# AaltoML/free-hunch

Measured on AMD Instinct MI355X. Metric: images/sec (256x256, num_steps=30, FH-Heun), higher is better.
Workload: dtype f32 UNet (convolutions: exact 3-way bf16 split on the bf16 MFMA, fp32 accuracy) + f64 covariance/CG; 1 GPU; FFHQ-256 arch, gaussian_blur, FH low-rank covariance (dct_diagonal), num_steps=30 heun, batch=8 per GPU; lockstep_groups_per_gpu=2, unet_backend=hip, net_calls_per_image=59

## Files before the change

free-hunch_amd/_lib.py:

```python
from __future__ import annotations

import ctypes as C
import os

import torch

_HERE = os.path.dirname(os.path.abspath(__file__))
LIB_PATH = os.path.join(_HERE, "libfh_hip.so")

c_dp = C.c_void_p


class FhProblem(C.Structure):
    _fields_ = [("op", C.c_int32), ("use_dct", C.c_int32), ("planes", C.c_int32), ("stride", C.c_int32),
                ("ntaps", C.c_int32), ("m", C.c_int32), ("ldm", C.c_int32), ("halo", C.c_int32),
                ("d", C.c_int64), ("sigma_y2", C.c_double),
                ("tap_dy", c_dp), ("tap_dx", c_dp), ("tap_w", c_dp), ("mask", c_dp),
                ("D", c_dp), ("r", c_dp), ("B", c_dp), ("M", c_dp),
                ("ntaps2", C.c_int32), ("halo2", C.c_int32), ("cg_scipy", C.c_int32), ("fold_sym", C.c_int32),
                ("tap2_dy", c_dp), ("tap2_dx", c_dp), ("tap2_w", c_dp),
                ("fold_fwd_w", c_dp), ("fold_fwd_h", c_dp), ("fold_inv_w", c_dp), ("fold_inv_h", c_dp)]


FH_MAX_BATCH = 16
# ... 56 lines not shown
    "fh_amm": ([C.c_void_p, C.POINTER(FhProblem), c_dp, c_dp, C.c_void_p], C.c_int),
    "fh_dense_matvec_scratch_doubles": ([C.c_int, C.c_int64], C.c_int64),
    "fh_dense_matvec": ([c_dp, c_dp, c_dp, c_dp, C.c_int, C.c_int64, C.c_int, C.c_double, C.c_double, C.c_void_p], C.c_int),
    "fh_dense_rank2": ([c_dp, c_dp, C.c_int, C.c_int64, c_dp, c_dp, c_dp, c_dp, c_dp, c_dp, C.c_double, C.c_double,
                        C.c_void_p], C.c_int),
    "fh_conv2d_nhwc": ([c_dp, c_dp, c_dp, c_dp, c_dp, c_dp] + [C.c_int] * 10 + [C.c_void_p], C.c_int),
    "fh_conv2d_x6_nhwc": ([c_dp, c_dp, c_dp, c_dp, c_dp, c_dp] + [C.c_int] * 10 + [C.c_void_p], C.c_int),
    "fh_conv2d_x6_nhwc_gn": ([c_dp, c_dp, c_dp, c_dp, c_dp, c_dp] + [C.c_int] * 10 + [C.POINTER(FhGnEpilogue), C.c_void_p],
                             C.c_int),
    "fh_conv2d_x6_gn_chunks": ([C.c_int] * 10, C.c_int),
    "fh_groupnorm_finalize": ([c_dp, c_dp, C.c_int, C.c_int, C.c_double, C.c_int, C.c_void_p], C.c_int),
    "fh_groupnorm_bwd_table": ([c_dp, c_dp, c_dp, c_dp, c_dp, C.c_int, c_dp, C.c_int, C.c_int, C.c_void_p], C.c_int),
    "fh_groupnorm_bwd_apply": ([c_dp] * 8 + [C.c_int, c_dp] + [C.c_int] * 5 + [C.c_void_p], C.c_int),
    "fh_groupnorm_bwd_sums": ([c_dp] * 7 + [C.c_int, c_dp, c_dp] + [C.c_int] * 4 + [C.c_void_p], C.c_int),
    "fh_groupnorm_bwd_apply_ex": ([c_dp] * 8 + [C.c_int, c_dp, c_dp, c_dp, c_dp] + [C.c_int] * 5 + [c_dp, C.c_void_p], C.c_int),
    "fh_conv2d_splitk": ([C.c_int] * 7, C.c_int),
    "fh_unet_set_precision": ([C.c_int], C.c_int),
    "fh_unet_get_precision": ([], C.c_int),
    "fh_absmax_f32": ([c_dp, C.c_int64, c_dp, C.c_void_p], C.c_int),
    "fh_groupnorm_table": ([c_dp, c_dp, c_dp, c_dp, c_dp, C.c_int, c_dp, C.c_int, C.c_int, C.c_void_p], C.c_int),
    "fh_conv2d_x6_norm_supported": ([C.c_int] * 5, C.c_int),
    "fh_conv2d_x6_norm_nhwc": ([c_dp, c_dp, C.c_int, c_dp, c_dp, c_dp, c_dp] + [C.c_int] * 5 + [C.c_void_p], C.c_int),
    "fh_conv2d_x6_norm_nhwc_gn": ([c_dp, c_dp, C.c_int, c_dp, c_dp, c_dp, c_dp] + [C.c_int] * 5
                                  + [C.POINTER(FhGnEpilogue), C.c_void_p], C.c_int),
    "fh_conv3x3_thin_nhwc": ([c_dp, c_dp, c_dp, c_dp] + [C.c_int] * 5 + [C.c_void_p], C.c_int),
    "fh_conv3x3_wino_nhwc": ([c_dp, c_dp, c_dp, c_dp, c_dp] + [C.c_int] * 5 + [C.c_void_p], C.c_int),
    "fh_bgemm_f32": ([c_dp, c_dp, c_dp] + [C.c_int] * 10 + [C.c_int64] * 6 + [C.c_float, C.c_void_p], C.c_int),
    "fh_groupnorm_scratch_doubles": ([C.c_int, C.c_int], C.c_int64),
    "fh_groupnorm_stats": ([c_dp, c_dp, c_dp, C.c_int, C.c_int, C.c_int, C.c_void_p], C.c_int),
    "fh_groupnorm_apply": ([c_dp] * 6 + [C.c_int, c_dp, C.c_int, C.c_int, C.c_int, C.c_int, C.c_void_p], C.c_int),
# ... 138 lines not shown
```

free-hunch_amd/csrc/fh_unet.hip:

```cpp
#include "fh_common.h"
#include <stdlib.h>

typedef float float16_t __attribute__((ext_vector_type(16)));

namespace {

constexpr int kBK = 32;
constexpr int kLd = kBK + 4;

struct ConvArgs {
  const float* in;
  const float* w;
  const float* bias;
  const float* res;
  float* out;
  int N, H, W, Cin, Cout, KH, KW, pad, stride, Ho, Wo;
  int ksplit;
  float* ws;
};

__device__ __forceinline__ void xcd_tile(int& tile_m, int& tile_n) {
  const unsigned gx = gridDim.x, gy = gridDim.y;
  const unsigned total = gx * gy;
  unsigned lin = blockIdx.y * gx + blockIdx.x;
// ... 1052 lines not shown
  if (col < g.N) {
#pragma unroll
    for (int r = 0; r < 16; ++r) {
      const int row = m0 + wm + (r & 3) + 8 * (r >> 2) + 4 * lh;
      if (row < g.M) C[(int64_t)row * g.ldc + col] = g.alpha * acc[r];
    }
  }
}

static inline int gn_chunk(int N, int P) {
  int c = 512;
  while (c > 32 && (int64_t)N * ((P + c - 1) / c) < 256) c >>= 1;
  return c;
}

template <int MODE>
__global__ __launch_bounds__(256) void k_gn_partial(const float* __restrict__ x, const float* __restrict__ dy,
                                                    const float* __restrict__ stats, const float* __restrict__ gamma,
                                                    const float* __restrict__ beta, const float* __restrict__ scale,
                                                    const float* __restrict__ shift, int ss_stride,
                                                    double* __restrict__ partial, int P, int C, int act, int nchunks,
                                                    int kGnChunk) {
  __shared__ double acc[64];
  const int n = blockIdx.x / nchunks, chunk = blockIdx.x % nchunks;
  const int cg = C / 32, c4n = C / 4;
  if (threadIdx.x < 64) acc[threadIdx.x] = 0.0;
  __syncthreads();
  const int p0 = chunk * kGnChunk;
  const int p1 = p0 + kGnChunk < P ? p0 + kGnChunk : P;
  const int lanes_p = c4n >= 256 ? 1 : 256 / c4n;
  const int active = c4n >= 256 ? 256 : lanes_p * c4n;
  if ((int)threadIdx.x < active) {
    for (int c4 = threadIdx.x % (c4n < 256 ? c4n : 256); c4 < c4n; c4 += 256) {
      const int psub = c4n >= 256 ? 0 : threadIdx.x / c4n;
      double s0[4] = {0, 0, 0, 0}, s1[4] = {0, 0, 0, 0};
      float ga[4], be[4], sc[4], sh[4], mean[4], rstd[4];
      if (MODE == 1) {
#pragma unroll
        for (int e = 0; e < 4; ++e) {
          const int c = 4 * c4 + e;
          ga[e] = gamma[c], be[e] = beta[c];
          sc[e] = scale != nullptr ? 1.f + scale[(int64_t)n * ss_stride + c] : 1.f;
          sh[e] = shift != nullptr ? shift[(int64_t)n * ss_stride + c] : 0.f;
          mean[e] = stats[((int64_t)n * 32 + c / cg) * 2], rstd[e] = stats[((int64_t)n * 32 + c / cg) * 2 + 1];
        }
      }
      for (int pb = p0 + psub; pb < p1; pb += 4 * lanes_p) {
        float4 xv[4], gv[4];
        bool ok[4];
#pragma unroll
        for (int u = 0; u < 4; ++u) {
          const int p = pb + u * lanes_p;
          ok[u] = p < p1;
          const int64_t idx = ((int64_t)n * P + (ok[u] ? p : p0)) * C + 4 * c4;
          xv[u] = *reinterpret_cast<const float4*>(x + idx);
          if (MODE == 1) gv[u] = *reinterpret_cast<const float4*>(dy + idx);
        }
#pragma unroll
        for (int u = 0; u < 4; ++u) {
          if (!ok[u]) continue;
          const float xs[4] = {xv[u].x, xv[u].y, xv[u].z, xv[u].w};
          if (MODE == 0) {
#pragma unroll
            for (int e = 0; e < 4; ++e) {
              s0[e] += xs[e];
              s1[e] += (double)xs[e] * xs[e];
            }
          } else {
            const float gs[4] = {gv[u].x, gv[u].y, gv[u].z, gv[u].w};
#pragma unroll
            for (int e = 0; e < 4; ++e) {
              const float xh = (xs[e] - mean[e]) * rstd[e];
              const float t = (xh * ga[e] + be[e]) * sc[e] + sh[e];
              float g = gs[e];
// ... 40 lines not shown
  for (int g = 0; g < 16; ++g) s += red[g][slot];
  const int grp = slot >> 1, which = slot & 1;
  const double other = __shfl_xor(s, 1, 64);
  if (MODE == 1) {
    out[((int64_t)n * 32 + grp) * 2 + which] = (float)(s / count);
  } else {
    const double sum = which ? other : s, sq = which ? s : other;
    const double mean = sum / count;
    double var = sq / count - mean * mean;
    var = var < 0 ? 0 : var;
    out[((int64_t)n * 32 + grp) * 2 + which] = which ? (float)(1.0 / sqrt(var + 1e-5)) : (float)mean;
  }
}


typedef float f4v_t __attribute__((ext_vector_type(4)));
__device__ __forceinline__ float4 ld_stream(const float* p, int nt) {
  if (nt) {
    const f4v_t v = __builtin_nontemporal_load(reinterpret_cast<const f4v_t*>(p));
    return make_float4(v.x, v.y, v.z, v.w);
  }
  return *reinterpret_cast<const float4*>(p);
}

template <int BWD, bool AMAX = false>
__global__ __launch_bounds__(256) void k_gn_stream(const float* __restrict__ x, const float* __restrict__ dy,
                                                   const float* __restrict__ stats, const float* __restrict__ sums,
                                                   const float* __restrict__ gamma, const float* __restrict__ beta,
                                                   const float* __restrict__ scale, const float* __restrict__ shift,
                                                   int ss_stride, float* __restrict__ out, int P, int C, int act,
                                                   int accumulate, int nchunks, int kGnChunk,
                                                   const float* __restrict__ acc_src = nullptr,
                                                   const float* __restrict__ add2 = nullptr, float* __restrict__ out2 = nullptr,
                                                   int csplit = 0, unsigned* __restrict__ amax = nullptr, int nt = 0) {
  unsigned mx0 = 0u, mx1 = 0u;
  const int n = blockIdx.x / nchunks, chunk = blockIdx.x % nchunks;
  const int cg = C / 32, c4n = C / 4;
  const int p0 = chunk * kGnChunk;
  const int p1 = p0 + kGnChunk < P ? p0 + kGnChunk : P;
  const int lanes_p = c4n >= 256 ? 1 : 256 / c4n;
  const int active = c4n >= 256 ? 256 : lanes_p * c4n;
  const bool live = (int)threadIdx.x < active;
  if (!live && !(BWD && AMAX)) return;
  for (int c4 = threadIdx.x % (c4n < 256 ? c4n : 256); live && c4 < c4n; c4 += 256) {
    const int psub = c4n >= 256 ? 0 : threadIdx.x / c4n;
    float A[4], Bc[4], mean[4], rstd[4], gsc[4], sa[4], sb[4];
#pragma unroll
    for (int e = 0; e < 4; ++e) {
      const int c = 4 * c4 + e;
      const int64_t si = ((int64_t)n * 32 + c / cg) * 2;
      mean[e] = stats[si], rstd[e] = stats[si + 1];
      const float sc = scale != nullptr ? 1.f + scale[(int64_t)n * ss_stride + c] : 1.f;
      const float sh = shift != nullptr ? shift[(int64_t)n * ss_stride + c] : 0.f;
      const float rg = rstd[e] * gamma[c];
      A[e] = rg * sc;
      Bc[e] = (beta[c] - mean[e] * rg) * sc + sh;
      gsc[e] = sc * gamma[c];
      if (BWD) sa[e] = sums[si], sb[e] = sums[si + 1];
    }
    for (int pb = p0 + psub; pb < p1; pb += 4 * lanes_p) {
      float4 xv[4], gv[4], ov[4];
      bool ok[4];
#pragma unroll
      for (int u = 0; u < 4; ++u) {
        const int p = pb + u * lanes_p;
        ok[u] = p < p1;
        const int64_t idx = ((int64_t)n * P + (ok[u] ? p : p0)) * C + 4 * c4;
        xv[u] = *reinterpret_cast<const float4*>(x + idx);
        if (BWD) {
          gv[u] = ld_stream(dy + idx, nt);
          if (accumulate) ov[u] = ld_stream((acc_src != nullptr ? acc_src : out) + idx, nt);
          if (add2 != nullptr) {
            const float4 t2 = ld_stream(add2 + idx, nt);
            if (accumulate)
              ov[u].x += t2.x, ov[u].y += t2.y, ov[u].z += t2.z, ov[u].w += t2.w;
            else
              ov[u] = t2;
          }
        }
      }
#pragma unroll
      for (int u = 0; u < 4; ++u) {
        if (!ok[u]) continue;
        const int64_t idx = ((int64_t)n * P + pb + u * lanes_p) * C + 4 * c4;
        const float xs[4] = {xv[u].x, xv[u].y, xv[u].z, xv[u].w};
        float o[4];
        if (!BWD) {
#pragma unroll
          for (int e = 0; e < 4; ++e) {
            const float t = fmaf(xs[e], A[e], Bc[e]);
            o[e] = act ? silu_f(t) : t;
          }
        } else {
          const float gs[4] = {gv[u].x, gv[u].y, gv[u].z, gv[u].w};
          const float os[4] = {ov[u].x, ov[u].y, ov[u].z, ov[u].w};
#pragma unroll
          for (int e = 0; e < 4; ++e) {
// ... 99 lines not shown
      reinterpret_cast<float4*>(out)[i] = v;
    }
  }
}

__global__ __launch_bounds__(256) void k_concat(float* __restrict__ a, float* __restrict__ b, float* __restrict__ out,
                                                int64_t P, int Ca, int Cb, int split) {
  const int C4 = (Ca + Cb) / 4, Ca4 = Ca / 4, Cb4 = Cb / 4;
  for (int64_t i = (int64_t)blockIdx.x * 256 + threadIdx.x; i < P * C4; i += (int64_t)gridDim.x * 256) {
    const int c4 = (int)(i % C4);
    const int64_t p = i / C4;
    float4* o = reinterpret_cast<float4*>(out) + i;
    float4* s = c4 < Ca4 ? reinterpret_cast<float4*>(a) + p * Ca4 + c4 : reinterpret_cast<float4*>(b) + p * Cb4 + (c4 - Ca4);
    if (split) *s = *o; else *o = *s;
  }
}

__global__ __launch_bounds__(256) void k_nchw_to_nhwc(const float* __restrict__ in, float* __restrict__ out, int N,
                                                      int C, int64_t P, int Cp) {
  for (int64_t i = (int64_t)blockIdx.x * 256 + threadIdx.x; i < (int64_t)N * P * Cp; i += (int64_t)gridDim.x * 256) {
    const int c = (int)(i % Cp);
    const int64_t p = (i / Cp) % P, n = i / (Cp * P);
    out[i] = c < C ? in[((int64_t)n * C + c) * P + p] : 0.f;
  }
}
__global__ __launch_bounds__(256) void k_nhwc_to_nchw(const float* __restrict__ in, float* __restrict__ out, int N,
                                                      int C, int64_t P, int Cp) {
  for (int64_t i = (int64_t)blockIdx.x * 256 + threadIdx.x; i < (int64_t)N * C * P; i += (int64_t)gridDim.x * 256) {
    const int64_t p = i % P;
    const int c = (int)((i / P) % C);
// ... 103 lines not shown
  }
  return false;
}

bool launch_x6_tile(const X6Plan& p, hipStream_t st, const ConvArgsX& a) {
  switch (tile_key(p.bm, p.bn)) {
    case tile_key(128, 128): launch_x6<2, 1, 2, 4, 4>(p, st, a); return true;
    case tile_key(64, 128): launch_x6<1, 2, 2, 2, 2>(p, st, a); return true;
    case tile_key(64, 64): launch_x6<1, 1, 2, 2, 2>(p, st, a); return true;
  }
  return false;
}

}

extern "C" {

int fh_unet_set_precision(int mode) {
  if (mode < 0 || mode > 4) return FH_EINVAL;
  g_conv_np = mode == 0 ? 3 : (mode == 1 ? 1 : (mode == 2 ? 2 : (mode == 3 ? 16 : 32)));
  return 0;
}

int fh_unet_get_precision(void) {
  return g_conv_np == 3 ? 0 : (g_conv_np == 1 ? 1 : (g_conv_np == 2 ? 2 : (g_conv_np == 16 ? 3 : 4)));
}

int fh_absmax_f32(const float* x, int64_t n, float* out, void* stream) {
  if (!out || n < 0 || (n > 0 && !x) || ((uintptr_t)x & 15)) return FH_EINVAL;
  hipStream_t st = (hipStream_t)stream;
// ... 335 lines not shown
  const int nchunks = (P + kGnChunk - 1) / kGnChunk;
  static const int nt_env = getenv("FH_GN_NT") ? atoi(getenv("FH_GN_NT")) : 1;
  const int nt = nt_env && (int64_t)N * P * C * 4 > ((int64_t)200 << 20);
  if (amax2 != nullptr)
    hipLaunchKernelGGL((k_gn_stream<1, true>), dim3(N * nchunks), dim3(256), 0, (hipStream_t)stream, x, dy, stats, sums, gamma,
                       beta, scale, shift, ss_stride, dx, P, C, act, acc_src != nullptr ? 1 : 0, nchunks, kGnChunk, acc_src, add2,
                       dx2, csplit, reinterpret_cast<unsigned*>(amax2), nt);
  else
    hipLaunchKernelGGL((k_gn_stream<1, false>), dim3(N * nchunks), dim3(256), 0, (hipStream_t)stream, x, dy, stats, sums, gamma,
                       beta, scale, shift, ss_stride, dx, P, C, act, acc_src != nullptr ? 1 : 0, nchunks, kGnChunk, acc_src, add2,
                       dx2, csplit, (unsigned*)nullptr, nt);
  FH_LAUNCH_CHECK();
  return 0;
}

int fh_softmax_rows(float* s, int64_t rows, int T, void* stream) {
  if (!s || rows < 1 || T < 1) return FH_EINVAL;
  hipLaunchKernelGGL(k_softmax_rows, dim3((unsigned)rows), dim3(256), 0, (hipStream_t)stream, s, T);
  FH_LAUNCH_CHECK();
  return 0;
}

int fh_softmax_bwd_rows(const float* p, float* dp, int64_t rows, int T, void* stream) {
  if (!p || !dp || rows < 1 || T < 1) return FH_EINVAL;
  hipLaunchKernelGGL(k_softmax_bwd_rows, dim3((unsigned)rows), dim3(256), 0, (hipStream_t)stream, p, dp, T);
  FH_LAUNCH_CHECK();
  return 0;
}

int fh_resample2x(const float* in, float* out, int N, int Hs, int Ws, int C, int mode, void* stream) {
// ... 36 lines not shown
```

free-hunch_amd/unet_hip.py:

```python
from __future__ import annotations

import math
import os
import threading

import torch
import torch.nn.functional as F

import ctypes as C

from . import _lib

_K = 32


def _pad_to(n, m):
    return (n + m - 1) // m * m


def _wino(w):
    w0, w1, w2 = w[:, :, 0], w[:, :, 1], w[:, :, 2]
    return torch.stack([w0, (w0 + w1 + w2) / 2, (w0 - w1 + w2) / 2, w2], 0).contiguous()


# ... 209 lines not shown
        e.partial, e.mode, e.act = partial.data_ptr(), mode, 0
        e.in_amax = None if amax is None else amax.data_ptr()
        keep = [partial, chunks]
        if mode == 1:
            gn_name, x, stats, act, scale, shift = gn
            table = torch.empty(N, 5, Co, dtype=torch.float32, device=dev)
            ss = 0 if scale is None else scale.stride(0)
            _lib.check(self.lib.fh_groupnorm_bwd_table(
                stats.data_ptr(), self.P[gn_name + ".weight"].data_ptr(), self.P[gn_name + ".bias"].data_ptr(),
                None if scale is None else scale.data_ptr(), None if shift is None else shift.data_ptr(), ss,
                table.data_ptr(), N, Co, _lib.stream()), "gn_bwd_table")
            e.x, e.tab, e.act = x.data_ptr(), table.data_ptr(), int(act)
            keep.append(table)
        return C.byref(e), keep

    def _gn_stats(self, x):
        N, H, W, C_ = x.shape
        pre = getattr(x, "_fh_gn", None)
        if pre is not None:
            stats = torch.empty(N, 32, 2, dtype=torch.float32, device=x.device)
            _lib.check(self.lib.fh_groupnorm_finalize(pre[0].data_ptr(), stats.data_ptr(), N, pre[1],
                                                      float(H * W * (C_ // 32)), 0, _lib.stream()), "gn_finalize(0)")
            return stats
        return self._gn_stats_pass(x)

    def _gn_stats_pass(self, x):
        N, H, W, C = x.shape
        stats = torch.empty(N, 32, 2, dtype=torch.float32, device=x.device)
        scratch = torch.empty(self.lib.fh_groupnorm_scratch_doubles(N, H * W), dtype=torch.float64, device=x.device)
        _lib.check(self.lib.fh_groupnorm_stats(x.data_ptr(), stats.data_ptr(), scratch.data_ptr(), N, H * W, C,
# ... 1 lines not shown
        return stats

    def _gn_apply(self, name, x, stats, act, scale=None, shift=None):
        N, H, W, C = x.shape
        y = torch.empty_like(x)
        ss = 0 if scale is None else scale.stride(0)
        _lib.check(self.lib.fh_groupnorm_apply(
            x.data_ptr(), stats.data_ptr(), self.P[name + ".weight"].data_ptr(), self.P[name + ".bias"].data_ptr(),
            None if scale is None else scale.data_ptr(), None if shift is None else shift.data_ptr(), ss,
            y.data_ptr(), N, H * W, C, int(act), _lib.stream()), "gn_apply")
        return y

    def _gn(self, name, x, act, scale=None, shift=None):
        stats = self._gn_stats(x)
        return self._gn_apply(name, x, stats, act, scale, shift), stats

    def _gn_conv(self, gn_name, conv_name, x, act, scale=None, shift=None, res=None):
        c = self.conv[conv_name]
        N, H, W, Ci = x.shape
        stats = self._gn_stats(x)
        if (c.wx_f is not None and c.kh == 3 and c.kw == 3 and Ci == c.ci_p and os.environ.get("FH_GN_FUSE", "1") != "0"
                and self.lib.fh_conv2d_x6_norm_supported(N, H, W, Ci, c.co)):
            table = torch.empty(N, 2, Ci, dtype=torch.float32, device=x.device)
            ss = 0 if scale is None else scale.stride(0)
            _lib.check(self.lib.fh_groupnorm_table(
                stats.data_ptr(), self.P[gn_name + ".weight"].data_ptr(), self.P[gn_name + ".bias"].data_ptr(),
                None if scale is None else scale.data_ptr(), None if shift is None else shift.data_ptr(), ss,
                table.data_ptr(), N, Ci, _lib.stream()), "gn_table")
            out = torch.empty(N, H, W, c.co, dtype=torch.float32, device=x.device)
            epi, keep = self._epilogue(1, N, H, W, Ci, c.co, 3, 3, 1, 0)
            _lib.check(self.lib.fh_conv2d_x6_norm_nhwc_gn(x.data_ptr(), table.data_ptr(), int(act),
                                                          c.planes(True, self._launch_mode(c)).data_ptr(),
                                                          c.b.data_ptr(), None if res is None else res.data_ptr(),
                                                          out.data_ptr(), N, H, W, Ci, c.co, epi, _lib.stream()),
                       "fh_conv2d_x6_norm_nhwc")
            if keep is not None:
                out._fh_gn = keep
            return out, stats
        return self._conv(conv_name, self._gn_apply(gn_name, x, stats, act, scale, shift), res=res), stats

    def _gn_bwd(self, name, x, stats, dy, act, scale=None, shift=None, accumulate_into=None, add2=None, split=None):
        N, H, W, C_ = x.shape
        ss = 0 if scale is None else scale.stride(0)
        gp = (self.P[name + ".weight"].data_ptr(), self.P[name + ".bias"].data_ptr(),
              None if scale is None else scale.data_ptr(), None if shift is None else shift.data_ptr(), ss)
        sums = getattr(dy, "_fh_gn_sums", None)
        if sums is None:
            sums = torch.empty(N, 32, 2, dtype=torch.float32, device=x.device)
            scratch = torch.empty(self.lib.fh_groupnorm_scratch_doubles(N, H * W), dtype=torch.float64, device=x.device)
            _lib.check(self.lib.fh_groupnorm_bwd_sums(x.data_ptr(), dy.data_ptr(), stats.data_ptr(), *gp, sums.data_ptr(),
                                                      scratch.data_ptr(), N, H * W, C_, int(act), _lib.stream()), "gn_bwd_sums")
        acc = accumulate_into
        if split is not None:
            dx = torch.empty(N, H, W, split[0], dtype=torch.float32, device=x.device)
            dx2 = torch.empty(N, H, W, split[1], dtype=torch.float32, device=x.device)
        else:
            dx, dx2 = (acc if acc is not None else torch.empty_like(x)), None
        amax = self._amax_slot() if self.bf16 == 4 else None
        _lib.check(self.lib.fh_groupnorm_bwd_apply_ex(
            x.data_ptr(), dy.data_ptr(), stats.data_ptr(), sums.data_ptr(), *gp, None if acc is None else acc.data_ptr(),
            None if add2 is None else add2.data_ptr(), dx.data_ptr(), None if dx2 is None else dx2.data_ptr(),
            0 if split is None else split[0], N, H * W, C_, int(act), None if amax is None else amax.data_ptr(),
            _lib.stream()), "gn_bwd_apply")
        if amax is not None:
            dx._fh_amax = amax[0]
            if dx2 is not None:
                dx2._fh_amax = amax[1]
        return dx if split is None else (dx, dx2)

    def _resample(self, x, mode):
        N, H, W, C = x.shape
        hs, ws = (H // 2, W // 2) if mode in (0, 3) else (H, W)
        oh, ow = (hs, ws) if mode in (0, 3) else (2 * H, 2 * W)
        out = torch.empty(N, oh, ow, C, dtype=torch.float32, device=x.device)
        _lib.check(self.lib.fh_resample2x(x.data_ptr(), out.data_ptr(), N, hs, ws, C, mode, _lib.stream()), "resample")
        return out

    def _add(self, a, b):
# ... 13 lines not shown
            e = F.linear(F.silu(emb), self.P[prefix + ".emb_layers.1.weight"], self.P[prefix + ".emb_layers.1.bias"])
            e = e.float().contiguous()
            if ek is not None:
                if len(self._emb_cache) > 4096:
                    self._emb_cache.clear()
                self._emb_cache[key] = e
        return e

    def _res_fwd(self, op, p, x, emb, tape):
        cfg = self.cfg
        e = self.emb_out(p, emb)
        co = self.conv[p + ".in_layers.2"].co
        xs = x
        h0 = None
        if op != "res":
            h0, st0 = self._gn(p + ".in_layers.0", x, act=1)
            mode = 0 if op == "res_down" else 2
            h0, xs = self._resample(h0, mode), self._resample(x, mode)
        if cfg.use_scale_shift_norm:
            if h0 is None:
                h1, st0 = self._gn_conv(p + ".in_layers.0", p + ".in_layers.2", x, act=1)
            else:
                h1 = self._conv(p + ".in_layers.2", h0)
            scale, shift = e[:, :co], e[:, co:]
        else:
            if e.shape[0] != 1 and not bool((e == e[:1]).all()):
                raise NotImplementedError("per-sample timestep embeddings without scale-shift norm")
            if h0 is None:
                h0, st0 = self._gn(p + ".in_layers.0", x, act=1)
            h1 = self._conv(p + ".in_layers.2", h0, bias_override=(self.conv[p + ".in_layers.2"].b + e[0]).contiguous())
            scale = shift = None
        skip = self._conv(p + ".skip_connection", xs) if (p + ".skip_connection") in self.conv else xs
        out, st1 = self._gn_conv(p + ".out_layers.0", p + ".out_layers.3", h1, act=1, scale=scale, shift=shift, res=skip)
        tape.append(("res", op, p, x, st0, h1, st1, scale, shift))
        return out

    def _res_bwd(self, rec, g, add2=None, split=None):
        _, op, p, x, st0, h1, st1, scale, shift = rec
        g_h2 = self._dgrad(p + ".out_layers.3", g, gn=(p + ".out_layers.0", h1, st1, 1, scale, shift))
        g_h1 = self._gn_bwd(p + ".out_layers.0", h1, st1, g_h2, 1, scale, shift)
        g_h0 = self._dgrad(p + ".in_layers.2", g_h1, gn=(p + ".in_layers.0", x, st0, 1, None, None) if op == "res" else None)
        g_xs = self._dgrad(p + ".skip_connection", g) if (p + ".skip_connection") in self.conv else g
        if op == "res_down":
            g_h0, g_xs = self._resample(g_h0, 1), self._resample(g_xs, 1)
        elif op == "res_up":
            g_h0, g_xs = self._resample(g_h0, 3), self._resample(g_xs, 3)
        return self._gn_bwd(p + ".in_layers.0", x, st0, g_h0, 1, accumulate_into=g_xs, add2=add2, split=split)

    def _attn_geometry(self, N, T, C, heads):
        ch = C // heads
        if self.cfg.use_new_attention_order:
            hs, qo, ko, vo = ch, 0, C, 2 * C
        else:
            hs, qo, ko, vo = 3 * ch, 0, ch, 2 * ch
        return ch, hs, qo, ko, vo

    def _attn_fwd(self, p, x, heads, tape):
        N, H, W, C = x.shape
        T = H * W
        hn, st = self._gn(p + ".norm", x, act=0)
        qkv = self._conv(p + ".qkv", hn)
        if (os.environ.get("FH_ATTN_FUSED", "1") != "0" and self.lib.fh_attention_supported(T, C, heads)
# ... 55 lines not shown
        st = _lib.stream()
        self.lib.fh_unet_set_precision(int(self.bf16))
        x = torch.empty(N, H, W, _pad_to(Cin, _K), dtype=torch.float32, device=x_nchw.device)
        _lib.check(self.lib.fh_layout_nchw_nhwc(x_nchw.contiguous().data_ptr(), x.data_ptr(), N, Cin, H * W, x.shape[-1],
                                                1, st), "layout")
        tape, stack, h = [], [], x
        for op, p, _ci, _co, heads in steps:
            if op == "push":
                stack.append(h)
                tape.append(("push",))
            elif op == "pop_cat":
                s = stack.pop()
                Nn, Hh, Ww, Ca = h.shape
                Cb = s.shape[-1]
                out = torch.empty(Nn, Hh, Ww, Ca + Cb, dtype=torch.float32, device=h.device)
                _lib.check(self.lib.fh_concat_channels(h.data_ptr(), s.data_ptr(), out.data_ptr(), Nn * Hh * Ww, Ca, Cb,
                                                       0, st), "concat")
                tape.append(("pop_cat", Ca, Cb))
                h = out
            elif op == "conv_in":
                h = self._conv(p, h)
                tape.append(("conv", p))
            elif op in ("res", "res_down", "res_up"):
                h = self._res_fwd(op, p, h, emb, tape)
            elif op == "attn":
                h = self._attn_fwd(p, h, heads, tape)
            elif op == "down":
                if cfg.conv_resample:
                    h = self._conv(p + ".op", h, stride=2)
                    tape.append(("down_conv", p + ".op"))
                else:
                    h = self._resample(h, 0)
# ... 14 lines not shown
        return out, tape

    def backward_tape(self, tape, g_nchw):
        N, Co, H, W = g_nchw.shape
        st = _lib.stream()
        self.lib.fh_unet_set_precision(int(self.bf16))
        self._tls.amax_pool = None
        cp = self.conv["out.2"].co_p
        g = torch.empty(N, H, W, cp, dtype=torch.float32, device=g_nchw.device)
        _lib.check(self.lib.fh_layout_nchw_nhwc(g_nchw.contiguous().data_ptr(), g.data_ptr(), N, Co, H * W, cp, 1, st),
                   "layout")
        pending = []
        recs = list(reversed(tape))
        presplit = None
        skip_push = False
        fold = os.environ.get("FH_GLUE_FOLD", "1") != "0"
        for ri, rec in enumerate(recs):
            kind = rec[0]
            nxt = recs[ri + 1] if ri + 1 < len(recs) else (None,)
            if kind == "out":
                _, h, stn = rec
                g = self._dgrad("out.2", g)
                g = self._gn_bwd("out.0", h, stn, g, 1)
            elif kind in ("res", "attn"):
                add2 = pending.pop() if (fold and nxt[0] == "push") else None
                skip_push = add2 is not None
                if kind == "res":
                    split = (nxt[1], nxt[2]) if (fold and nxt[0] == "pop_cat" and nxt[1] % 4 == 0) else None
                    g = self._res_bwd(rec, g, add2=add2, split=split)
                    if split is not None:
                        presplit, g = g, None
                else:
                    g = self._attn_bwd(rec, g, add2=add2)
            elif kind == "pop_cat":
                _, Ca, Cb = rec
                if presplit is not None:
                    ga, gb = presplit
# ... 47 lines not shown
```

include/fh_hip.h:

```cpp
#ifndef FH_HIP_H
#define FH_HIP_H

#include <stdint.h>

#ifdef __cplusplus
extern "C" {
#endif

#define FH_EINVAL (-1)
#define FH_ESYNC (-3)
#define FH_ESIZE (-2)
#define FH_MAX_COLS 256

typedef struct fh_context fh_context;

int fh_version(void);
int fh_context_create(fh_context** out, int S, int planes_max, int m_cap);
int fh_context_destroy(fh_context* ctx);
int fh_context_set_exclusive(fh_context* ctx, int exclusive);
int fh_context_status(fh_context* ctx, void* stream);
int fh_debug_read_stamps(fh_context* ctx, unsigned long long* out_host, int count, void* stream);

int fh_dct2d(fh_context* ctx, const double* in, double* out, int planes, int inverse, void* stream);

// ... 154 lines not shown
                              void* stream);
int fh_groupnorm_finalize(const double* partial, float* out, int N, int chunks, double count, int mode, void* stream);
int fh_groupnorm_bwd_table(const float* stats, const float* gamma, const float* beta, const float* scale, const float* shift,
                           int ss_stride, float* table, int N, int C, void* stream);
int fh_groupnorm_bwd_apply(const float* x, const float* dy, const float* stats, const float* sums, const float* gamma,
                           const float* beta, const float* scale, const float* shift, int ss_stride, float* dx, int N, int P,
                           int C, int act, int accumulate, void* stream);
int fh_groupnorm_bwd_sums(const float* x, const float* dy, const float* stats, const float* gamma, const float* beta,
                          const float* scale, const float* shift, int ss_stride, float* sums, double* scratch, int N, int P,
                          int C, int act, void* stream);
int fh_groupnorm_bwd_apply_ex(const float* x, const float* dy, const float* stats, const float* sums, const float* gamma,
                              const float* beta, const float* scale, const float* shift, int ss_stride, const float* acc_src,
                              const float* add2, float* dx, float* dx2, int csplit, int N, int P, int C, int act, float* amax2,
                              void* stream);

int fh_conv3x3_thin_nhwc(const float* in, const float* w, const float* bias, float* out, int N, int H, int W, int Cin,
                         int Cout, void* stream);

int fh_conv3x3_wino_nhwc(const float* in, const float* wu, const float* bias, const float* res, float* out, int N,
                         int H, int W, int Cin, int Cout, void* stream);

int fh_bgemm_f32(const float* A, const float* B, float* C, int M, int N, int K, int lda, int ldb, int ldc, int transA,
                 int transB, int batch, int inner, int64_t sA0, int64_t sA1, int64_t sB0, int64_t sB1, int64_t sC0,
                 int64_t sC1, float alpha, void* stream);

int64_t fh_groupnorm_scratch_doubles(int N, int P);
int fh_groupnorm_stats(const float* x, float* stats, double* scratch, int N, int P, int C, void* stream);
int fh_groupnorm_apply(const float* x, const float* stats, const float* gamma, const float* beta, const float* scale,
                       const float* shift, int ss_stride, float* y, int N, int P, int C, int act, void* stream);
int fh_groupnorm_bwd(const float* x, const float* dy, const float* stats, const float* gamma, const float* beta,
// ... 47 lines not shown
```

Before: 2.409 images/s.

## Fuse groupnorm with down/up resampling and concat with GN stats in UNet glue

Adds kernels that fuse GroupNorm apply+SiLU with the 2x average-pool or nearest upsample of both the activation and the skip input. The GN backward kernels now read resampled gradients directly through index mapping. The concat kernel also accumulates GN partial statistics while writing the output, and the output layer's dgrad gets the GN fusion. Together these remove several intermediate full-resolution tensors and separate elementwise passes, at the cost of more kernel variants and indexed gather loads. The up-path backward still materializes one resample.

```diff
diff --git a/free-hunch_amd/_lib.py b/free-hunch_amd/_lib.py
--- a/free-hunch_amd/_lib.py
+++ b/free-hunch_amd/_lib.py
@@ -94,6 +94,10 @@
     "fh_groupnorm_bwd_apply": ([c_dp] * 8 + [C.c_int, c_dp] + [C.c_int] * 5 + [C.c_void_p], C.c_int),
     "fh_groupnorm_bwd_sums": ([c_dp] * 7 + [C.c_int, c_dp, c_dp] + [C.c_int] * 4 + [C.c_void_p], C.c_int),
     "fh_groupnorm_bwd_apply_ex": ([c_dp] * 8 + [C.c_int, c_dp, c_dp, c_dp, c_dp] + [C.c_int] * 5 + [c_dp, C.c_void_p], C.c_int),
+    "fh_groupnorm_apply_resample": ([c_dp] * 6 + [C.c_int, c_dp, c_dp] + [C.c_int] * 6 + [C.c_void_p], C.c_int),
+    "fh_groupnorm_bwd_sums_rs": ([c_dp] * 7 + [C.c_int, c_dp, c_dp] + [C.c_int] * 6 + [C.c_void_p], C.c_int),
+    "fh_groupnorm_bwd_apply_rs": ([c_dp] * 8 + [C.c_int, c_dp, c_dp, c_dp, c_dp] + [C.c_int] * 8 + [c_dp, C.c_void_p], C.c_int),
+    "fh_concat_channels_stats": ([c_dp] * 4 + [C.c_int] * 4 + [C.c_void_p], C.c_int),
     "fh_conv2d_splitk": ([C.c_int] * 7, C.c_int),
     "fh_unet_set_precision": ([C.c_int], C.c_int),
     "fh_unet_get_precision": ([], C.c_int),
diff --git a/free-hunch_amd/csrc/fh_unet.hip b/free-hunch_amd/csrc/fh_unet.hip
--- a/free-hunch_amd/csrc/fh_unet.hip
+++ b/free-hunch_amd/csrc/fh_unet.hip
@@ -1090,13 +1090,38 @@
   return c;
 }
 
-template <int MODE>
+typedef float f4v_t __attribute__((ext_vector_type(4)));
+__device__ __forceinline__ float4 ld_stream(const float* p, int nt) {
+  if (nt) {
+    const f4v_t v = __builtin_nontemporal_load(reinterpret_cast<const f4v_t*>(p));
+    return make_float4(v.x, v.y, v.z, v.w);
+  }
+  return *reinterpret_cast<const float4*>(p);
+}
+
+template <int RS>
+__device__ __forceinline__ float4 ld_resampled(const float* g, int n, int p, int H, int W, int C, int c0, int nt) {
+#pragma clang fp contract(off)
+  const int h = p / W, w = p - h * W;
+  if (RS == 1) {
+    const float4 v = *reinterpret_cast<const float4*>(g + (((int64_t)n * (H / 2) + h / 2) * (W / 2) + w / 2) * C + c0);
+    return make_float4(0.25f * v.x, 0.25f * v.y, 0.25f * v.z, 0.25f * v.w);
+  }
+  const int64_t row = (int64_t)2 * W * C;
+  const float* s = g + (((int64_t)n * 2 * H + 2 * h) * 2 * W + 2 * w) * C + c0;
+  const float4 a = ld_stream(s, nt), b = ld_stream(s + C, nt), c = ld_stream(s + row, nt), d = ld_stream(s + row + C, nt);
+  return make_float4(((a.x + b.x) + c.x) + d.x, ((a.y + b.y) + c.y) + d.y, ((a.z + b.z) + c.z) + d.z,
+                     ((a.w + b.w) + c.w) + d.w);
+}
+
+template <int MODE, int RS = 0>
 __global__ __launch_bounds__(256) void k_gn_partial(const float* __restrict__ x, const float* __restrict__ dy,
                                                     const float* __restrict__ stats, const float* __restrict__ gamma,
                                                     const float* __restrict__ beta, const float* __restrict__ scale,
                                                     const float* __restrict__ shift, int ss_stride,
                                                     double* __restrict__ partial, int P, int C, int act, int nchunks,
-                                                    int kGnChunk) {
+                                                    int kGnChunk, int H = 0, int W = 0) {
+  constexpr int U = RS == 3 ? 2 : 4;
   __shared__ double acc[64];
   const int n = blockIdx.x / nchunks, chunk = blockIdx.x % nchunks;
   const int cg = C / 32, c4n = C / 4;
@@ -1121,19 +1146,24 @@
           mean[e] = stats[((int64_t)n * 32 + c / cg) * 2], rstd[e] = stats[((int64_t)n * 32 + c / cg) * 2 + 1];
         }
       }
-      for (int pb = p0 + psub; pb < p1; pb += 4 * lanes_p) {
-        float4 xv[4], gv[4];
-        bool ok[4];
-#pragma unroll
-        for (int u = 0; u < 4; ++u) {
+      for (int pb = p0 + psub; pb < p1; pb += U * lanes_p) {
+        float4 xv[U], gv[U];
+        bool ok[U];
+#pragma unroll
+        for (int u = 0; u < U; ++u) {
           const int p = pb + u * lanes_p;
           ok[u] = p < p1;
           const int64_t idx = ((int64_t)n * P + (ok[u] ? p : p0)) * C + 4 * c4;
           xv[u] = *reinterpret_cast<const float4*>(x + idx);
-          if (MODE == 1) gv[u] = *reinterpret_cast<const float4*>(dy + idx);
-        }
-#pragma unroll
-        for (int u = 0; u < 4; ++u) {
+          if (MODE == 1) {
+            if (RS)
+              gv[u] = ld_resampled<RS>(dy, n, ok[u] ? p : p0, H, W, C, 4 * c4, 0);
+            else
+              gv[u] = *reinterpret_cast<const float4*>(dy + idx);
+          }
+        }
+#pragma unroll
+        for (int u = 0; u < U; ++u) {
           if (!ok[u]) continue;
           const float xs[4] = {xv[u].x, xv[u].y, xv[u].z, xv[u].w};
           if (MODE == 0) {
@@ -1204,16 +1234,8 @@
 }
 
 
-typedef float f4v_t __attribute__((ext_vector_type(4)));
-__device__ __forceinline__ float4 ld_stream(const float* p, int nt) {
-  if (nt) {
-    const f4v_t v = __builtin_nontemporal_load(reinterpret_cast<const f4v_t*>(p));
-    return make_float4(v.x, v.y, v.z, v.w);
-  }
-  return *reinterpret_cast<const float4*>(p);
-}
-
-template <int BWD, bool AMAX = false>
+
+template <int BWD, bool AMAX = false, int RS = 0>
 __global__ __launch_bounds__(256) void k_gn_stream(const float* __restrict__ x, const float* __restrict__ dy,
                                                    const float* __restrict__ stats, const float* __restrict__ sums,
                                                    const float* __restrict__ gamma, const float* __restrict__ beta,
@@ -1222,7 +1244,9 @@
                                                    int accumulate, int nchunks, int kGnChunk,
                                                    const float* __restrict__ acc_src = nullptr,
                                                    const float* __restrict__ add2 = nullptr, float* __restrict__ out2 = nullptr,
-                                                   int csplit = 0, unsigned* __restrict__ amax = nullptr, int nt = 0) {
+                                                   int csplit = 0, unsigned* __restrict__ amax = nullptr, int nt = 0,
+                                                   int H = 0, int W = 0, int dy_mapped = 1) {
+  constexpr int U = RS == 3 ? 2 : 4;
   unsigned mx0 = 0u, mx1 = 0u;
   const int n = blockIdx.x / nchunks, chunk = blockIdx.x % nchunks;
   const int cg = C / 32, c4n = C / 4;
@@ -1248,18 +1272,24 @@
       gsc[e] = sc * gamma[c];
       if (BWD) sa[e] = sums[si], sb[e] = sums[si + 1];
     }
-    for (int pb = p0 + psub; pb < p1; pb += 4 * lanes_p) {
-      float4 xv[4], gv[4], ov[4];
-      bool ok[4];
-#pragma unroll
-      for (int u = 0; u < 4; ++u) {
+    for (int pb = p0 + psub; pb < p1; pb += U * lanes_p) {
+      float4 xv[U], gv[U], ov[U];
+      bool ok[U];
+#pragma unroll
+      for (int u = 0; u < U; ++u) {
         const int p = pb + u * lanes_p;
         ok[u] = p < p1;
         const int64_t idx = ((int64_t)n * P + (ok[u] ? p : p0)) * C + 4 * c4;
         xv[u] = *reinterpret_cast<const float4*>(x + idx);
-        if (BWD) {
+        if (BWD && RS) {
+          const int pc = ok[u] ? p : p0;
+          gv[u] = dy_mapped ? ld_resampled<RS>(dy, n, pc, H, W, C, 4 * c4, nt) : ld_stream(dy + idx, nt);
+          if (accumulate) ov[u] = ld_resampled<RS>(acc_src, n, pc, H, W, C, 4 * c4, nt);
+        } else if (BWD) {
           gv[u] = ld_stream(dy + idx, nt);
           if (accumulate) ov[u] = ld_stream((acc_src != nullptr ? acc_src : out) + idx, nt);
+        }
+        if (BWD) {
           if (add2 != nullptr) {
             const float4 t2 = ld_stream(add2 + idx, nt);
             if (accumulate)
@@ -1270,7 +1300,7 @@
         }
       }
 #pragma unroll
-      for (int u = 0; u < 4; ++u) {
+      for (int u = 0; u < U; ++u) {
         if (!ok[u]) continue;
         const int64_t idx = ((int64_t)n * P + pb + u * lanes_p) * C + 4 * c4;
         const float xs[4] = {xv[u].x, xv[u].y, xv[u].z, xv[u].w};
@@ -1400,6 +1430,151 @@
     float4* s = c4 < Ca4 ? reinterpret_cast<float4*>(a) + p * Ca4 + c4 : reinterpret_cast<float4*>(b) + p * Cb4 + (c4 - Ca4);
     if (split) *s = *o; else *o = *s;
   }
+}
+
+__device__ __forceinline__ float pool4(float a, float b, float c, float d) {
+#pragma clang fp contract(off)
+  return 0.25f * (((a + b) + c) + d);
+}
+
+template <int MODE>
+__global__ __launch_bounds__(256) void k_gn_stream_resample(const float* __restrict__ x, const float* __restrict__ stats,
+                                                            const float* __restrict__ gamma, const float* __restrict__ beta,
+                                                            const float* __restrict__ scale, const float* __restrict__ shift,
+                                                            int ss_stride, float* __restrict__ out_y, float* __restrict__ out_x,
+                                                            int Hs, int Ws, int C, int act, int nchunks, int kGnChunk) {
+  constexpr int U = MODE == 0 ? 2 : 4;
+  constexpr int Q = MODE == 0 ? 4 : 1;
+  const int n = blockIdx.x / nchunks, chunk = blockIdx.x % nchunks;
+  const int cg = C / 32, c4n = C / 4, P = Hs * Ws;
+  const int p0 = chunk * kGnChunk;
+  const int p1 = p0 + kGnChunk < P ? p0 + kGnChunk : P;
+  const int lanes_p = c4n >= 256 ? 1 : 256 / c4n;
+  const int active = c4n >= 256 ? 256 : lanes_p * c4n;
+  if ((int)threadIdx.x >= active) return;
+  const int64_t row = (int64_t)2 * Ws * C;
+  for (int c4 = threadIdx.x % (c4n < 256 ? c4n : 256); c4 < c4n; c4 += 256) {
+    const int psub = c4n >= 256 ? 0 : threadIdx.x / c4n;
+    float A[4], Bc[4];
+#pragma unroll
+    for (int e = 0; e < 4; ++e) {
+      const int c = 4 * c4 + e;
+      const int64_t si = ((int64_t)n * 32 + c / cg) * 2;
+      const float mean = stats[si], rstd = stats[si + 1];
+      const float sc = scale != nullptr ? 1.f + scale[(int64_t)n * ss_stride + c] : 1.f;
+      const float sh = shift != nullptr ? shift[(int64_t)n * ss_stride + c] : 0.f;
+      const float rg = rstd * gamma[c];
+      A[e] = rg * sc;
+      Bc[e] = (beta[c] - mean * rg) * sc + sh;
+    }
+    for (int pb = p0 + psub; pb < p1; pb += U * lanes_p) {
+      float4 xv[U][Q];
+      int64_t big[U];
+      bool ok[U];
+#pragma unroll
+      for (int u = 0; u < U; ++u) {
+        const int p = pb + u * lanes_p;
+        ok[u] = p < p1;
+        const int pc = ok[u] ? p : p0;
+        const int hs = pc / Ws, ws = pc - hs * Ws;
+        big[u] = (((int64_t)n * 2 * Hs + 2 * hs) * 2 * Ws + 2 * ws) * C + 4 * c4;
+        if constexpr (MODE == 0) {
+          const float* s = x + big[u];
+          xv[u][0] = *reinterpret_cast<const float4*>(s);
+          xv[u][1] = *reinterpret_cast<const float4*>(s + C);
+          xv[u][2] = *reinterpret_cast<const float4*>(s + row);
+          xv[u][3] = *reinterpret_cast<const float4*>(s + row + C);
+        } else {
+          xv[u][0] = *reinterpret_cast<const float4*>(x + ((int64_t)n * P + pc) * C + 4 * c4);
+        }
+      }
+#pragma unroll
+      for (int u = 0; u < U; ++u) {
+        if (!ok[u]) continue;
+        float xs[Q][4], ys[Q][4];
+#pragma unroll
+        for (int q = 0; q < Q; ++q) {
+          xs[q][0] = xv[u][q].x, xs[q][1] = xv[u][q].y, xs[q][2] = xv[u][q].z, xs[q][3] = xv[u][q].w;
+#pragma unroll
+          for (int e = 0; e < 4; ++e) {
+            const float t = fmaf(xs[q][e], A[e], Bc[e]);
+            ys[q][e] = act ? silu_f(t) : t;
+          }
+        }
+        if constexpr (MODE == 0) {
+          const int64_t o = ((int64_t)n * P + pb + u * lanes_p) * C + 4 * c4;
+          float py[4], px[4];
+#pragma unroll
+          for (int e = 0; e < 4; ++e) {
+            py[e] = pool4(ys[0][e], ys[1][e], ys[2][e], ys[3][e]);
+            px[e] = pool4(xs[0][e], xs[1][e], xs[2][e], xs[3][e]);
+          }
+          *reinterpret_cast<float4*>(out_y + o) = make_float4(py[0], py[1], py[2], py[3]);
+          *reinterpret_cast<float4*>(out_x + o) = make_float4(px[0], px[1], px[2], px[3]);
+        } else {
+          const float4 yv = make_float4(ys[0][0], ys[0][1], ys[0][2], ys[0][3]);
+          float* dy_ = out_y + big[u];
+          float* dx_ = out_x + big[u];
+          *reinterpret_cast<float4*>(dy_) = yv, *reinterpret_cast<float4*>(dy_ + C) = yv;
+          *reinterpret_cast<float4*>(dy_ + row) = yv, *reinterpret_cast<float4*>(dy_ + row + C) = yv;
+          *reinterpret_cast<float4*>(dx_) = xv[u][0], *reinterpret_cast<float4*>(dx_ + C) = xv[u][0];
+          *reinterpret_cast<float4*>(dx_ + row) = xv[u][0], *reinterpret_cast<float4*>(dx_ + row + C) = xv[u][0];
+        }
+      }
+    }
+  }
+}
+
+__global__ __launch_bounds__(256) void k_concat_stats(const float* __restrict__ a, const float* __restrict__ b,
+                                                      float* __restrict__ out, double* __restrict__ partial, int P, int Ca,
+                                                      int Cb, int nchunks, int kGnChunk) {
+  __shared__ double acc[64];
+  const int n = blockIdx.x / nchunks, chunk = blockIdx.x % nchunks;
+  const int C = Ca + Cb, cg = C / 32, c4n = C / 4;
+  if (threadIdx.x < 64) acc[threadIdx.x] = 0.0;
+  __syncthreads();
+  const int p0 = chunk * kGnChunk;
+  const int p1 = p0 + kGnChunk < P ? p0 + kGnChunk : P;
+  const int lanes_p = c4n >= 256 ? 1 : 256 / c4n;
+  const int active = c4n >= 256 ? 256 : lanes_p * c4n;
+  if ((int)threadIdx.x < active) {
+    for (int c4 = threadIdx.x % (c4n < 256 ? c4n : 256); c4 < c4n; c4 += 256) {
+      const int psub = c4n >= 256 ? 0 : threadIdx.x / c4n;
+      const bool in_a = 4 * c4 < Ca;
+      const float* src = in_a ? a + 4 * c4 : b + (4 * c4 - Ca);
+      const int sC = in_a ? Ca : Cb;
+      double s0[4] = {0, 0, 0, 0}, s1[4] = {0, 0, 0, 0};
+      for (int pb = p0 + psub; pb < p1; pb += 4 * lanes_p) {
+        float4 xv[4];
+        bool ok[4];
+#pragma unroll
+        for (int u = 0; u < 4; ++u) {
+          const int p = pb + u * lanes_p;
+          ok[u] = p < p1;
+          xv[u] = *reinterpret_cast<const float4*>(src + ((int64_t)n * P + (ok[u] ? p : p0)) * sC);
+        }
+#pragma unroll
+        for (int u = 0; u < 4; ++u) {
+          if (!ok[u]) continue;
+          *reinterpret_cast<float4*>(out + ((int64_t)n * P + pb + u * lanes_p) * C + 4 * c4) = xv[u];
+          const float xs[4] = {xv[u].x, xv[u].y, xv[u].z, xv[u].w};
+#pragma unroll
+          for (int e = 0; e < 4; ++e) {
+            s0[e] += xs[e];
+            s1[e] += (double)xs[e] * xs[e];
+          }
+        }
+      }
+#pragma unroll
+      for (int e = 0; e < 4; ++e) {
+        const int grp = (4 * c4 + e) / cg;
+        atomicAdd(&acc[2 * grp], s0[e]);
+        atomicAdd(&acc[2 * grp + 1], s1[e]);
+      }
+    }
+  }
+  __syncthreads();
+  if (threadIdx.x < 64) partial[(int64_t)blockIdx.x * 64 + threadIdx.x] = acc[threadIdx.x];
 }
 
 __global__ __launch_bounds__(256) void k_nchw_to_nhwc(const float* __restrict__ in, float* __restrict__ out, int N,
@@ -1533,6 +1708,18 @@
 
 }
 
+template <bool AMAX, int RS>
+static void launch_gn_stream_rs(const float* x, const float* dy, const float* stats, const float* sums, const float* gamma,
+                                const float* beta, const float* scale, const float* shift, int ss_stride, const float* acc_src,
+                                const float* add2, float* dx, float* dx2, int csplit, int N, int H, int W, int C, int act,
+                                int dy_mapped, float* amax2, int nt, hipStream_t st) {
+  const int P = H * W, kGnChunk = gn_chunk(N, P);
+  const int nchunks = (P + kGnChunk - 1) / kGnChunk;
+  hipLaunchKernelGGL((k_gn_stream<1, AMAX, RS>), dim3(N * nchunks), dim3(256), 0, st, x, dy, stats, sums, gamma, beta, scale,
+                     shift, ss_stride, dx, P, C, act, acc_src != nullptr ? 1 : 0, nchunks, kGnChunk, acc_src, add2, dx2, csplit,
+                     reinterpret_cast<unsigned*>(amax2), nt, H, W, dy_mapped);
+}
+
 extern "C" {
 
 int fh_unet_set_precision(int mode) {
@@ -1898,6 +2085,81 @@
   return 0;
 }
 
+int fh_groupnorm_apply_resample(const float* x, const float* stats, const float* gamma, const float* beta, const float* scale,
+                                const float* shift, int ss_stride, float* y_rs, float* x_rs, int N, int H, int W, int C,
+                                int act, int mode, void* stream) {
+  if (!x || !stats || !gamma || !beta || !y_rs || !x_rs || N < 1 || H < 1 || W < 1 || C % 32 != 0) return FH_EINVAL;
+  if (mode != 0 && mode != 2) return FH_EINVAL;
+  if (mode == 0 && ((H | W) & 1)) return FH_EINVAL;
+  const int Hs = mode == 0 ? H / 2 : H, Ws = mode == 0 ? W / 2 : W;
+  const int kGnChunk = gn_chunk(N, Hs * Ws);
+  const int nchunks = (Hs * Ws + kGnChunk - 1) / kGnChunk;
+  if (mode == 0)
+    hipLaunchKernelGGL(k_gn_stream_resample<0>, dim3(N * nchunks), dim3(256), 0, (hipStream_t)stream, x, stats, gamma, beta,
+                       scale, shift, ss_stride, y_rs, x_rs, Hs, Ws, C, act, nchunks, kGnChunk);
+  else
+    hipLaunchKernelGGL(k_gn_stream_resample<2>, dim3(N * nchunks), dim3(256), 0, (hipStream_t)stream, x, stats, gamma, beta,
+                       scale, shift, ss_stride, y_rs, x_rs, Hs, Ws, C, act, nchunks, kGnChunk);
+  FH_LAUNCH_CHECK();
+  return 0;
+}
+
+static bool rs_shape_ok(int N, int H, int W, int C, int mode) {
+  return N >= 1 && H >= 1 && W >= 1 && C % 32 == 0 && (mode == 3 || (mode == 1 && !((H | W) & 1)));
+}
+
+int fh_groupnorm_bwd_sums_rs(const float* x, const float* dy, const float* stats, const float* gamma, const float* beta,
+                             const float* scale, const float* shift, int ss_stride, float* sums, double* scratch, int N, int H,
+                             int W, int C, int act, int mode, void* stream) {
+  if (!x || !dy || !stats || !gamma || !beta || !sums || !scratch || !rs_shape_ok(N, H, W, C, mode)) return FH_EINVAL;
+  hipStream_t st = (hipStream_t)stream;
+  const int P = H * W, kGnChunk = gn_chunk(N, P);
+  const int nchunks = (P + kGnChunk - 1) / kGnChunk;
+  if (mode == 1)
+    hipLaunchKernelGGL((k_gn_partial<1, 1>), dim3(N * nchunks), dim3(256), 0, st, x, dy, stats, gamma, beta, scale, shift,
+                       ss_stride, scratch, P, C, act, nchunks, kGnChunk, H, W);
+  else
+    hipLaunchKernelGGL((k_gn_partial<1, 3>), dim3(N * nchunks), dim3(256), 0, st, x, dy, stats, gamma, beta, scale, shift,
+                       ss_stride, scratch, P, C, act, nchunks, kGnChunk, H, W);
+  hipLaunchKernelGGL(k_gn_finalize<1>, dim3(N), dim3(1024), 0, st, (const double*)scratch, sums, nchunks,
+                     (double)P * (C / 32));
+  FH_LAUNCH_CHECK();
+  return 0;
+}
+
+int fh_groupnorm_bwd_apply_rs(const float* x, const float* dy, const float* stats, const float* sums, const float* gamma,
+                              const float* beta, const float* scale, const float* shift, int ss_stride, const float* acc_src,
+                              const float* add2, float* dx, float* dx2, int csplit, int N, int H, int W, int C, int act,
+                              int mode, int dy_mapped, float* amax2, void* stream) {
+  if (!x || !dy || !stats || !sums || !gamma || !beta || !dx || !rs_shape_ok(N, H, W, C, mode)) return FH_EINVAL;
+  if (dx2 != nullptr && (csplit <= 0 || csplit >= C || csplit % 4 != 0)) return FH_EINVAL;
+  if (dx == dy || dx == acc_src || (mode == 1 && !dy_mapped)) return FH_EINVAL;
+  hipStream_t st = (hipStream_t)stream;
+  const int nt = (int64_t)N * H * W * C * 4 > ((int64_t)200 << 20);
+#define FH_RS_ARGS x, dy, stats, sums, gamma, beta, scale, shift, ss_stride, acc_src, add2, dx, dx2, csplit, N, H, W, C, act, \
+                   dy_mapped, amax2, nt, st
+  if (mode == 1) {
+    if (amax2 != nullptr) launch_gn_stream_rs<true, 1>(FH_RS_ARGS); else launch_gn_stream_rs<false, 1>(FH_RS_ARGS);
+  } else {
+    if (amax2 != nullptr) launch_gn_stream_rs<true, 3>(FH_RS_ARGS); else launch_gn_stream_rs<false, 3>(FH_RS_ARGS);
+  }
+#undef FH_RS_ARGS
+  FH_LAUNCH_CHECK();
+  return 0;
+}
+
+int fh_concat_channels_stats(const float* a, const float* b, float* out, double* scratch, int N, int P, int Ca, int Cb,
+                             void* stream) {
+  if (!a || !b || !out || !scratch || N < 1 || P < 1 || Ca < 4 || Cb < 4 || Ca % 4 != 0 || Cb % 4 != 0 || (Ca + Cb) % 32 != 0)
+    return FH_EINVAL;
+  const int kGnChunk = gn_chunk(N, P);
+  const int nchunks = (P + kGnChunk - 1) / kGnChunk;
+  hipLaunchKernelGGL(k_concat_stats, dim3(N * nchunks), dim3(256), 0, (hipStream_t)stream, a, b, out, scratch, P, Ca, Cb,
+                     nchunks, kGnChunk);
+  FH_LAUNCH_CHECK();
+  return 0;
+}
+
 int fh_softmax_rows(float* s, int64_t rows, int T, void* stream) {
   if (!s || rows < 1 || T < 1) return FH_EINVAL;
   hipLaunchKernelGGL(k_softmax_rows, dim3((unsigned)rows), dim3(256), 0, (hipStream_t)stream, s, T);
diff --git a/free-hunch_amd/unet_hip.py b/free-hunch_amd/unet_hip.py
--- a/free-hunch_amd/unet_hip.py
+++ b/free-hunch_amd/unet_hip.py
@@ -247,6 +247,10 @@
             keep.append(table)
         return C.byref(e), keep
 
+    @staticmethod
+    def _glue_fold():
+        return os.environ.get("FH_GLUE_FOLD", "1") != "0"
+
     def _gn_stats(self, x):
         N, H, W, C_ = x.shape
         pre = getattr(x, "_fh_gn", None)
@@ -278,6 +282,17 @@
     def _gn(self, name, x, act, scale=None, shift=None):
         stats = self._gn_stats(x)
         return self._gn_apply(name, x, stats, act, scale, shift), stats
+
+    def _gn_resample(self, name, x, act, mode):
+        N, H, W, C = x.shape
+        stats = self._gn_stats(x)
+        oh, ow = (H // 2, W // 2) if mode == 0 else (2 * H, 2 * W)
+        y = torch.empty(N, oh, ow, C, dtype=torch.float32, device=x.device)
+        xr = torch.empty_like(y)
+        _lib.check(self.lib.fh_groupnorm_apply_resample(
+            x.data_ptr(), stats.data_ptr(), self.P[name + ".weight"].data_ptr(), self.P[name + ".bias"].data_ptr(), None, None,
+            0, y.data_ptr(), xr.data_ptr(), N, H, W, C, int(act), mode, _lib.stream()), "gn_apply_resample")
+        return y, xr, stats
 
     def _gn_conv(self, gn_name, conv_name, x, act, scale=None, shift=None, res=None):
         c = self.conv[conv_name]
@@ -303,7 +318,8 @@
             return out, stats
         return self._conv(conv_name, self._gn_apply(gn_name, x, stats, act, scale, shift), res=res), stats
 
-    def _gn_bwd(self, name, x, stats, dy, act, scale=None, shift=None, accumulate_into=None, add2=None, split=None):
+    def _gn_bwd(self, name, x, stats, dy, act, scale=None, shift=None, accumulate_into=None, add2=None, split=None, rs=0,
+                dy_mapped=True):
         N, H, W, C_ = x.shape
         ss = 0 if scale is None else scale.stride(0)
         gp = (self.P[name + ".weight"].data_ptr(), self.P[name + ".bias"].data_ptr(),
@@ -312,20 +328,30 @@
         if sums is None:
             sums = torch.empty(N, 32, 2, dtype=torch.float32, device=x.device)
             scratch = torch.empty(self.lib.fh_groupnorm_scratch_doubles(N, H * W), dtype=torch.float64, device=x.device)
-            _lib.check(self.lib.fh_groupnorm_bwd_sums(x.data_ptr(), dy.data_ptr(), stats.data_ptr(), *gp, sums.data_ptr(),
-                                                      scratch.data_ptr(), N, H * W, C_, int(act), _lib.stream()), "gn_bwd_sums")
+            if rs and dy_mapped:
+                _lib.check(self.lib.fh_groupnorm_bwd_sums_rs(x.data_ptr(), dy.data_ptr(), stats.data_ptr(), *gp, sums.data_ptr(),
+                                                             scratch.data_ptr(), N, H, W, C_, int(act), rs, _lib.stream()),
+                           "gn_bwd_sums_rs")
+            else:
+                _lib.check(self.lib.fh_groupnorm_bwd_sums(x.data_ptr(), dy.data_ptr(), stats.data_ptr(), *gp, sums.data_ptr(),
+                                                          scratch.data_ptr(), N, H * W, C_, int(act), _lib.stream()), "gn_bwd_sums")
         acc = accumulate_into
         if split is not None:
             dx = torch.empty(N, H, W, split[0], dtype=torch.float32, device=x.device)
             dx2 = torch.empty(N, H, W, split[1], dtype=torch.float32, device=x.device)
         else:
-            dx, dx2 = (acc if acc is not None else torch.empty_like(x)), None
+            dx, dx2 = (acc if (acc is not None and not rs) else torch.empty_like(x)), None
         amax = self._amax_slot() if self.bf16 == 4 else None
-        _lib.check(self.lib.fh_groupnorm_bwd_apply_ex(
-            x.data_ptr(), dy.data_ptr(), stats.data_ptr(), sums.data_ptr(), *gp, None if acc is None else acc.data_ptr(),
-            None if add2 is None else add2.data_ptr(), dx.data_ptr(), None if dx2 is None else dx2.data_ptr(),
-            0 if split is None else split[0], N, H * W, C_, int(act), None if amax is None else amax.data_ptr(),
-            _lib.stream()), "gn_bwd_apply")
+        tail = (None if acc is None else acc.data_ptr(), None if add2 is None else add2.data_ptr(), dx.data_ptr(),
+                None if dx2 is None else dx2.data_ptr(), 0 if split is None else split[0])
+        if rs:
+            _lib.check(self.lib.fh_groupnorm_bwd_apply_rs(
+                x.data_ptr(), dy.data_ptr(), stats.data_ptr(), sums.data_ptr(), *gp, *tail, N, H, W, C_, int(act), rs,
+                int(dy_mapped), None if amax is None else amax.data_ptr(), _lib.stream()), "gn_bwd_apply_rs")
+        else:
+            _lib.check(self.lib.fh_groupnorm_bwd_apply_ex(
+                x.data_ptr(), dy.data_ptr(), stats.data_ptr(), sums.data_ptr(), *gp, *tail, N, H * W, C_, int(act),
+                None if amax is None else amax.data_ptr(), _lib.stream()), "gn_bwd_apply")
         if amax is not None:
             dx._fh_amax = amax[0]
             if dx2 is not None:
@@ -369,9 +395,12 @@
         xs = x
         h0 = None
         if op != "res":
-            h0, st0 = self._gn(p + ".in_layers.0", x, act=1)
             mode = 0 if op == "res_down" else 2
-            h0, xs = self._resample(h0, mode), self._resample(x, mode)
+            if self._glue_fold():
+                h0, xs, st0 = self._gn_resample(p + ".in_layers.0", x, 1, mode)
+            else:
+                h0, st0 = self._gn(p + ".in_layers.0", x, act=1)
+                h0, xs = self._resample(h0, mode), self._resample(x, mode)
         if cfg.use_scale_shift_norm:
             if h0 is None:
                 h1, st0 = self._gn_conv(p + ".in_layers.0", p + ".in_layers.2", x, act=1)
@@ -396,11 +425,17 @@
         g_h1 = self._gn_bwd(p + ".out_layers.0", h1, st1, g_h2, 1, scale, shift)
         g_h0 = self._dgrad(p + ".in_layers.2", g_h1, gn=(p + ".in_layers.0", x, st0, 1, None, None) if op == "res" else None)
         g_xs = self._dgrad(p + ".skip_connection", g) if (p + ".skip_connection") in self.conv else g
-        if op == "res_down":
+        rs, dy_mapped = 0, True
+        if op != "res" and self._glue_fold():
+            rs = 1 if op == "res_down" else 3
+            if rs == 3:
+                g_h0, dy_mapped = self._resample(g_h0, 3), False
+        elif op == "res_down":
             g_h0, g_xs = self._resample(g_h0, 1), self._resample(g_xs, 1)
         elif op == "res_up":
             g_h0, g_xs = self._resample(g_h0, 3), self._resample(g_xs, 3)
-        return self._gn_bwd(p + ".in_layers.0", x, st0, g_h0, 1, accumulate_into=g_xs, add2=add2, split=split)
+        return self._gn_bwd(p + ".in_layers.0", x, st0, g_h0, 1, accumulate_into=g_xs, add2=add2, split=split, rs=rs,
+                            dy_mapped=dy_mapped)
 
     def _attn_geometry(self, N, T, C, heads):
         ch = C // heads
@@ -486,8 +521,15 @@
                 Nn, Hh, Ww, Ca = h.shape
                 Cb = s.shape[-1]
                 out = torch.empty(Nn, Hh, Ww, Ca + Cb, dtype=torch.float32, device=h.device)
-                _lib.check(self.lib.fh_concat_channels(h.data_ptr(), s.data_ptr(), out.data_ptr(), Nn * Hh * Ww, Ca, Cb,
-                                                       0, st), "concat")
+                if self._glue_fold() and Ca % 4 == 0 and Cb % 4 == 0 and (Ca + Cb) % 32 == 0:
+                    nd = self.lib.fh_groupnorm_scratch_doubles(Nn, Hh * Ww)
+                    partial = torch.empty(nd, dtype=torch.float64, device=h.device)
+                    _lib.check(self.lib.fh_concat_channels_stats(h.data_ptr(), s.data_ptr(), out.data_ptr(), partial.data_ptr(),
+                                                                 Nn, Hh * Ww, Ca, Cb, st), "concat_stats")
+                    out._fh_gn = [partial, nd // (64 * Nn)]
+                else:
+                    _lib.check(self.lib.fh_concat_channels(h.data_ptr(), s.data_ptr(), out.data_ptr(), Nn * Hh * Ww, Ca, Cb,
+                                                           0, st), "concat")
                 tape.append(("pop_cat", Ca, Cb))
                 h = out
             elif op == "conv_in":
@@ -532,13 +574,13 @@
         recs = list(reversed(tape))
         presplit = None
         skip_push = False
-        fold = os.environ.get("FH_GLUE_FOLD", "1") != "0"
+        fold = self._glue_fold()
         for ri, rec in enumerate(recs):
             kind = rec[0]
             nxt = recs[ri + 1] if ri + 1 < len(recs) else (None,)
             if kind == "out":
                 _, h, stn = rec
-                g = self._dgrad("out.2", g)
+                g = self._dgrad("out.2", g, gn=("out.0", h, stn, 1, None, None) if fold else None)
                 g = self._gn_bwd("out.0", h, stn, g, 1)
             elif kind in ("res", "attn"):
                 add2 = pending.pop() if (fold and nxt[0] == "push") else None
diff --git a/include/fh_hip.h b/include/fh_hip.h
--- a/include/fh_hip.h
+++ b/include/fh_hip.h
@@ -192,6 +192,19 @@
                               const float* add2, float* dx, float* dx2, int csplit, int N, int P, int C, int act, float* amax2,
                               void* stream);
 
+int fh_groupnorm_apply_resample(const float* x, const float* stats, const float* gamma, const float* beta, const float* scale,
+                                const float* shift, int ss_stride, float* y_rs, float* x_rs, int N, int H, int W, int C,
+                                int act, int mode, void* stream);
+int fh_groupnorm_bwd_sums_rs(const float* x, const float* dy, const float* stats, const float* gamma, const float* beta,
+                             const float* scale, const float* shift, int ss_stride, float* sums, double* scratch, int N, int H,
+                             int W, int C, int act, int mode, void* stream);
+int fh_groupnorm_bwd_apply_rs(const float* x, const float* dy, const float* stats, const float* sums, const float* gamma,
+                              const float* beta, const float* scale, const float* shift, int ss_stride, const float* acc_src,
+                              const float* add2, float* dx, float* dx2, int csplit, int N, int H, int W, int C, int act,
+                              int mode, int dy_mapped, float* amax2, void* stream);
+int fh_concat_channels_stats(const float* a, const float* b, float* out, double* scratch, int N, int P, int Ca, int Cb,
+                             void* stream);
+
 int fh_conv3x3_thin_nhwc(const float* in, const float* w, const float* bias, float* out, int N, int H, int W, int Cin,
                          int Cout, void* stream);
 
```

Result: no change. 2.395 images/s (-0.6%).
